# sara-nl/2D-VQ-AE-2

Hardware: AMD Instinct MI355X
Metric: patches/sec (VQAE.forward: encoder -> VQ -> decoder) (higher is better)
Workload: dtype f32; 1 GPU; BASELINE configs[1] (cfg B): batch 256/GPU of 256x256x3 fp32 -> 32x32 codes, K=256, D=128, full forward; global_batch=256, parallelism=patch-sharded x1

## Files before the change

### 2d-vq-ae-2_amd/csrc/conv_wino.hip

```cpp
#include "kernels.h"
#include "mfma.h"

namespace {

using namespace vqae;

struct WinoK {
    const float* __restrict__ t1;
    const float* __restrict__ U;
    const float* __restrict__ w3;
    const float* __restrict__ w1n;
    float* xio;
    float* y2;
    int H, Wimg, M;
    float act_a, act_b, t_scale, t_b4, n_b1a, n_b1b, n_b2a, n_b2b;
};

constexpr int BPF = 6;

template <int C> struct WinoCfg {
    static constexpr int W = C >= 128 ? 32 : (C == 64 ? 64 : 128);
    static constexpr int NT = C == 256 ? 512 : 256;
    static constexpr int NW = NT / 64;
    static constexpr int PX = 4 * W;
    static constexpr int TILES = PX / 4;
    static constexpr int TC = W / 2;
    static constexpr int NS = C / 32;
    static constexpr int KS = C / 8;
    static constexpr int C4 = C / 4;
    static constexpr int RP = NT / C4;
    static constexpr int LDT = C + 4;
    static constexpr int NI = C >= 64 ? 2 : 1;
    static constexpr int WN = C / (32 * NI);
    static constexpr int MI = PX / ((NW / WN) * 32);
    static constexpr int LDS_BYTES = PX * LDT * 4;
    static constexpr int PREF = C <= 64 ? 1 : 0;
};

template <int C, int TAIL, int DT, bool WIDE>
__global__ __launch_bounds__((WinoCfg<C>::NT), 2)
void wino_trunk_kernel(const WinoK p) {
    using K = WinoCfg<C>;
    auto rnd = [](float v) -> float {
        if (DT == VQAE_DT_BF16) return (float)(__bf16)v;
        if (DT == VQAE_DT_F16) return (float)(_Float16)v;
        return v;
    };
    auto rnd4 = [&](f32x4 v) -> f32x4 {
        if (DT != VQAE_DT_F32) {
#pragma unroll
            for (int e = 0; e < 4; ++e) v[e] = rnd(v[e]);
        }
        return v;
    };
    constexpr int W = K::W, PX = K::PX, TC = K::TC, NS = K::NS, KS = K::KS, C4 = K::C4, RP = K::RP, LDT = K::LDT, WN = K::WN;
    constexpr int MI = K::MI, NI = K::NI;
    constexpr bool PREF = K::PREF && !WIDE;
// ... 57 lines not shown
        for (int s_c = 0; s_c < 2; ++s_c)
#pragma unroll
            for (int j = 0; j < 4; ++j)
                v[2 * s_r + s_c][j] = xi == 1 ? la[s_c][j] + lb[s_c][j] : la[s_c][j] - lb[s_c][j];
    };
    tr_load(0, 0);
    tr_combine(0, 0);
    tr_load(0, 1);
    tr_combine(0, 1);

    const int wm = wave / WN, wn = wave % WN;
    const int64_t pix0 = ((int64_t)img * p.H + row0) * Wimg + col0 + tj0;
    float* xr[4];
    f32x4 res[16];
    f32x4 bt[2][4][NI];
    auto tail_prefetch = [&](const float* __restrict__ wsrc) {
        const float* b0 = wsrc + (wn * NI) * (KS * 256) + 4 * lane;
#pragma unroll
        for (int u = 0; u < 4; ++u)
#pragma unroll
            for (int ni = 0; ni < NI; ++ni) bt[0][u][ni] = *reinterpret_cast<const f32x4*>(b0 + ni * (KS * 256) + 256 * u);
    };

    f32x16 y00, y01, y10, y11;
#pragma unroll
    for (int r = 0; r < 16; ++r) { y00[r] = 0.f; y01[r] = 0.f; y10[r] = 0.f; y11[r] = 0.f; }
#pragma unroll
    for (int xi = 0; xi < 4; ++xi) {
        __builtin_amdgcn_sched_barrier(0);
        if (xi > 0) __syncthreads();
#pragma unroll
        for (int it = 0; it < 4; ++it) {
            const int tile = (it >> 1) * TC + tj0 + RP * (it & 1);
            float* dst = lds + tile * LDT + 4 * cg;
            *reinterpret_cast<f32x4*>(dst + 0 * K::TILES * LDT) = v[it][0] - v[it][2];
            *reinterpret_cast<f32x4*>(dst + 1 * K::TILES * LDT) = v[it][1] + v[it][2];
            *reinterpret_cast<f32x4*>(dst + 2 * K::TILES * LDT) = v[it][2] - v[it][1];
            *reinterpret_cast<f32x4*>(dst + 3 * K::TILES * LDT) = v[it][1] - v[it][3];
        }

        const float* const ux = ub + (int64_t)(4 * xi) * (C * C);
#define WB(s) (((s) / KS) * (C * C) + 256 * ((s) % KS))
        f32x4 bq[BPF];
#pragma unroll
        for (int s = 0; s < BPF; ++s)
            bq[s] = *reinterpret_cast<const f32x4*>(ux + WB(s));
        __syncthreads();
        if (PREF && xi < 3) tr_load(xi + 1, 0);
        f32x4 aq[2];
        aq[0] = *reinterpret_cast<const f32x4*>(af);
#pragma unroll
        for (int nu = 0; nu < 4; ++nu) {
            f32x16 acc;
#pragma unroll
            for (int r = 0; r < 16; ++r) acc[r] = 0.f;
#pragma unroll
            for (int u = 0; u < KS; ++u) {
                const int s = KS * nu + u;
                if (s + 1 < STEPS)
                    aq[(s + 1) & 1] = *reinterpret_cast<const f32x4*>(af + ((s + 1) / KS) * K::TILES * LDT + 8 * ((s + 1) % KS));
                const f32x4 b = bq[s % BPF];
                if (s + BPF < STEPS)
                    bq[s % BPF] = *reinterpret_cast<const f32x4*>(ux + WB(s + BPF));
                if (xi == 3 && s == STEPS - BPF) {
                    tail_prefetch(p.w3);
#pragma unroll
                    for (int r = 0; r < 4; ++r) xr[r] = p.xio + (pix0 + (int64_t)r * Wimg) * C + 4 * cg;
#pragma unroll
                    for (int i = 0; i < 16; ++i) res[i] = __builtin_nontemporal_load(reinterpret_cast<const f32x4*>(xr[(RP * i) / W] + ((RP * i) % W) * C));
                }
#pragma unroll
                for (int r = 0; r < 4; ++r)
                    acc = __builtin_amdgcn_mfma_f32_32x32x2f32(b[r], aq[s & 1][r], acc, 0, 0, 0);
                __builtin_amdgcn_sched_barrier(0);
            }
            const int ca0 = xi <= 2 ? 1 : 0, ca1 = xi == 0 ? 0 : (xi == 1 ? 1 : -1);
            const int cb0 = nu <= 2 ? 1 : 0, cb1 = nu == 0 ? 0 : (nu == 1 ? 1 : -1);
            if (ca0 * cb0 != 0) y00 = y00 + acc;
            if (ca0 * cb1 == 1) y01 = y01 + acc; else if (ca0 * cb1 == -1) y01 = y01 - acc;
            if (ca1 * cb0 == 1) y10 = y10 + acc; else if (ca1 * cb0 == -1) y10 = y10 - acc;
            if (ca1 * cb1 == 1) y11 = y11 + acc; else if (ca1 * cb1 == -1) y11 = y11 - acc;
            asm volatile("" : "+v"(y00), "+v"(y01), "+v"(y10), "+v"(y11));
        }
#undef WB
        if (xi < 3) {
            if (!PREF) tr_load(xi + 1, 0);
            tr_combine(xi + 1, 0); tr_load(xi + 1, 1); tr_combine(xi + 1, 1);
        }
    }

    __syncthreads();
    float* const T = lds;
    {
        const int tile = mt * 32 + li;
        const int px = (2 * (tile / TC)) * W + 2 * (tile % TC);
        float* const d = T + px * LDT + 32 * ns + 4 * hh;
#pragma unroll
        for (int g = 0; g < 4; ++g) {
            f32x4 o00, o01, o10, o11;
#pragma unroll
            for (int e = 0; e < 4; ++e) {
                o00[e] = rnd(elu_act(rnd(y00[4 * g + e]) + p.act_a) + p.act_b);
                o01[e] = rnd(elu_act(rnd(y01[4 * g + e]) + p.act_a) + p.act_b);
                o10[e] = rnd(elu_act(rnd(y10[4 * g + e]) + p.act_a) + p.act_b);
// ... 4 lines not shown
            *reinterpret_cast<f32x4*>(d + 8 * g + W * LDT) = o10;
            *reinterpret_cast<f32x4*>(d + 8 * g + (W + 1) * LDT) = o11;
        }
    }
    __syncthreads();

    f32x16 acc[MI][NI];
    auto gemm_tail = [&](const float* __restrict__ wsrc) {
#pragma unroll
        for (int mi = 0; mi < MI; ++mi)
#pragma unroll
            for (int ni = 0; ni < NI; ++ni)
#pragma unroll
                for (int r = 0; r < 16; ++r) acc[mi][ni][r] = 0.f;
        const float* a0 = T + (wm * MI * 32 + li) * LDT + 4 * hh;
        const float* b0 = wsrc + (wn * NI) * (KS * 256) + 4 * lane;
        f32x4 a[2][MI];
#pragma unroll
        for (int mi = 0; mi < MI; ++mi) a[0][mi] = *reinterpret_cast<const f32x4*>(a0 + mi * 32 * LDT);
#pragma unroll
        for (int ug = 0; ug < KS / 4; ++ug) {
            if (ug + 1 < KS / 4) {
#pragma unroll
                for (int u = 0; u < 4; ++u)
#pragma unroll
                    for (int ni = 0; ni < NI; ++ni)
                        bt[(ug + 1) & 1][u][ni] = *reinterpret_cast<const f32x4*>(b0 + ni * (KS * 256) + 256 * (4 * (ug + 1) + u));
            }
#pragma unroll
            for (int u = 0; u < 4; ++u) {
// ... 256 lines not shown
#pragma unroll
    for (int a = 0; a < 4; ++a) {
        U[(a * 4 + 0) * cc + fo] = t[a][0];
        U[(a * 4 + 1) * cc + fo] = 0.5f * (t[a][0] + t[a][1] + t[a][2]);
        U[(a * 4 + 2) * cc + fo] = 0.5f * (t[a][0] - t[a][1] + t[a][2]);
        U[(a * 4 + 3) * cc + fo] = t[a][2];
    }
}

__global__ void frag_weight_kernel(const float* __restrict__ w, int n_rows, int K, int sk, float* __restrict__ out) {
    const int i = blockIdx.x * blockDim.x + threadIdx.x;
    if (i >= n_rows * K) return;
    out[frag_offset(i / K, i % K, K, sk)] = w[i];
}

template <int C, int DT, bool WIDE>
int launch_wino_w(const WinoK& k, bool chain, hipStream_t stream) {
    using K = WinoCfg<C>;
    if (int rc = vqae::set_max_dynamic_lds((const void*)wino_trunk_kernel<C, 1, DT, WIDE>, K::LDS_BYTES)) return rc;
    if (int rc = vqae::set_max_dynamic_lds((const void*)wino_trunk_kernel<C, 2, DT, WIDE>, K::LDS_BYTES)) return rc;
    const unsigned grid = (unsigned)(k.M / K::PX);
    const double flops = 2.0 * (double)k.M * C * (4.0 * C + C + (chain ? C : 0));
    vqae::ProfScope prof(C >= 128 ? vqae::PROF_CONV3X3_TRUNK : vqae::PROF_NONE, stream, flops);
    if (chain) wino_trunk_kernel<C, 2, DT, WIDE><<<grid, K::NT, K::LDS_BYTES, stream>>>(k);
    else wino_trunk_kernel<C, 1, DT, WIDE><<<grid, K::NT, K::LDS_BYTES, stream>>>(k);
    prof.done();
    VQAE_LAUNCH_CHECK();
    return VQAE_OK;
}

template <int C, int DT = VQAE_DT_F32>
int launch_wino(const WinoK& k, bool chain, hipStream_t stream) {
    return k.Wimg == WinoCfg<C>::W ? launch_wino_w<C, DT, false>(k, chain, stream) : launch_wino_w<C, DT, true>(k, chain, stream);
}

}

namespace vqae {

bool wino_trunk_channels(int c, int dtype) { return dtype == VQAE_DT_F32 ? (c == 256 || c == 128 || c == 64 || c == 32) : c == 32; }

bool wino_trunk_supported(int c, int h, int w, int dtype) {
    if (!wino_trunk_channels(c, dtype)) return false;
    const int span = c >= 128 ? 32 : (c == 64 ? WinoCfg<64>::W : WinoCfg<32>::W);
    return w >= span && w % span == 0 && h >= 4 && h % 4 == 0;
}

size_t wino_weight_floats(int c) { return (size_t)16 * c * c; }

int wino_transform_weight(const float* w_oihw_dev, int c, int dtype, float* U_dev, hipStream_t stream) {
    wino_weight_kernel<<<(unsigned)ceil_div(c * c, 256), 256, 0, stream>>>(w_oihw_dev, c, dtype, U_dev);
    VQAE_LAUNCH_CHECK();
    return VQAE_OK;
}

bool fixup_conv1_supported(int c, int64_t m) {
    if (c != 256 && c != 128 && c != 64 && c != 32) return false;
    const int px = c >= 128 ? 128 : (c == 64 ? WinoCfg<64>::PX : WinoCfg<32>::PX);
    return m > 0 && m % px == 0;
}

template <int C>
static int launch_conv1(const float* x, const float* w1f, float pa, float pb, float aa, float ab, float* y, int64_t m,
// ... 23 lines not shown
    VQAE_REQUIRE(m / 128 < (1ll << 31), VQAE_ERR_UNSUPPORTED, "fixup_conv1: too many pixels");
    if (c == 256) return launch_conv1<256>(x, w1f, pa, pb, aa, ab, y, m, stream);
    if (c == 128) return launch_conv1<128>(x, w1f, pa, pb, aa, ab, y, m, stream);
    if (c == 64) return launch_conv1<64>(x, w1f, pa, pb, aa, ab, y, m, stream);
    return launch_conv1<32>(x, w1f, pa, pb, aa, ab, y, m, stream);
}

int frag_weight(const float* w_packed_dev, int n_rows, int K, int sk, float* out_dev, hipStream_t stream) {
    VQAE_REQUIRE(n_rows % 32 == 0 && (sk == 8 || sk == 16) && K % sk == 0, VQAE_ERR_INVALID, "frag_weight: %d x %d, k-slice %d", n_rows, K, sk);
    frag_weight_kernel<<<(unsigned)ceil_div((int64_t)n_rows * K, 256), 256, 0, stream>>>(w_packed_dev, n_rows, K, sk, out_dev);
    VQAE_LAUNCH_CHECK();
    return VQAE_OK;
}

int wino_trunk_tail(const float* t1, const float* U, const float* w3, float act_a, float act_b, float t_scale, float t_b4,
                    float* xio, const NextConv1& next, int batch, int h, int w, int c, int dtype, hipStream_t stream) {
    if (batch == 0) return VQAE_OK;
    const float* w1n = (const float*)next.w1;
    float* t1_next = (float*)next.t1_next;
    VQAE_REQUIRE(t1 && U && w3 && xio && (!w1n || t1_next), VQAE_ERR_INVALID, "wino_trunk_tail: null pointer");
    VQAE_REQUIRE(wino_trunk_supported(c, h, w, dtype), VQAE_ERR_UNSUPPORTED, "wino_trunk_tail: C = %d, H = %d, W = %d, dtype %d", c, h, w, dtype);
    const int64_t M = (int64_t)batch * h * w;
    VQAE_REQUIRE(M < (1ll << 31) - 256, VQAE_ERR_UNSUPPORTED, "wino_trunk_tail: too many pixels");
    WinoK k;
    memset(&k, 0, sizeof(k));
    k.t1 = t1; k.U = U; k.w3 = w3; k.w1n = w1n; k.xio = xio; k.y2 = t1_next;
    k.H = h; k.Wimg = w; k.M = (int)M;
    k.act_a = act_a; k.act_b = act_b; k.t_scale = t_scale; k.t_b4 = t_b4;
    k.n_b1a = next.b1a; k.n_b1b = next.b1b; k.n_b2a = next.b2a; k.n_b2b = next.b2b;
    return dtype == VQAE_DT_BF16 ? launch_wino<32, VQAE_DT_BF16>(k, w1n != nullptr, stream)
         : dtype == VQAE_DT_F16 ? launch_wino<32, VQAE_DT_F16>(k, w1n != nullptr, stream)
         : c == 256 ? launch_wino<256>(k, w1n != nullptr, stream)
         : c == 128 ? launch_wino<128>(k, w1n != nullptr, stream)
         : (c == 64 ? launch_wino<64>(k, w1n != nullptr, stream) : launch_wino<32>(k, w1n != nullptr, stream));
}

}
```

### 2d-vq-ae-2_amd/csrc/handle.hip

```cpp
#include "kernels.h"

#include <algorithm>
#include <cmath>
#include <cstdlib>
#include <map>
#include <mutex>
#include <set>
#include <string>
#include <unordered_map>
#include <utility>
#include <vector>

namespace vqae {
char* last_error_buf() {
    static thread_local char buf[512] = {0};
    return buf;
}

ProfState& prof_state() {
    static ProfState p;
    return p;
}

int set_max_dynamic_lds(const void* kernel, int bytes) {
// ... 60 lines not shown
}

extern "C" const char* vqae_last_error(void) { return vqae::last_error_buf(); }
extern "C" const char* vqae_build_info(void) { return "gfx950;fp32-mfma;" __DATE__; }

namespace {

enum { MODE_SAME = 0, MODE_DOWN = 1, MODE_UP = 2 };

struct Block : vqae::FixupScalars {
    int mode, cin, cout, br;
    float *w1, *w2, *w3, *wskip;
    float* wU43 = nullptr;
    void *wU43s = nullptr, *w1s = nullptr, *w3s = nullptr;
    float* wU = nullptr;
    float *w1f = nullptr, *w3f = nullptr;
    float *w2f = nullptr, *wskf = nullptr;
    void *w1h = nullptr, *w2h = nullptr, *w3h = nullptr, *wskh = nullptr;
    int kind = VQAE_BLOCK_FIXUP, hidden = 0;
    float *bv1 = nullptr, *bv2 = nullptr, *bv3 = nullptr;
    float *fc0w = nullptr, *fc0b = nullptr, *fc2w = nullptr, *fc2b = nullptr;
};

const float kMean255[3] = {0.7279f * 255.0f, 0.5955f * 255.0f, 0.7762f * 255.0f};
const float kInv255[3] = {1.0f / (0.2419f * 255.0f), 1.0f / (0.3083f * 255.0f), 1.0f / (0.1741f * 255.0f)};
const float kStd255[3] = {0.2419f * 255.0f, 0.3083f * 255.0f, 0.1741f * 255.0f};

}

struct vqae_handle {
// ... 12 lines not shown
    size_t buf_floats = 0;
    void* vq_ws = nullptr;
    size_t vq_ws_bytes = 0;
    float* loss_scratch = nullptr;
    int device = 0;
    bool has_encoder = false, has_decoder = false;
    bool fuse_trunk = true;
    bool t1_ready = false;
    bool up_conv_first = true;
    bool fuse_down = true;
    bool fuse_down16 = true;
    bool fuse_up16 = true;
    bool fuse_up_tail = true;
    bool use_wino = true;
    bool w43_split = true;
    void* idx_scratch = nullptr;
    size_t idx_scratch_bytes = 0;
    float* se_ws = nullptr;
    size_t se_ws_bytes = 0;
    size_t se_gate_off = 0;
};

namespace {

using TensorMap = std::unordered_map<std::string, const vqae_tensor*>;

int find(const TensorMap& tm, const std::string& name, int64_t numel, const float** out) {
    auto it = tm.find(name);
    if (it == tm.end()) return vqae::fail(VQAE_ERR_NOT_FOUND, "missing tensor '%s'", name.c_str());
    if (it->second->numel != numel)
// ... 65 lines not shown
    return VQAE_OK;
}

int load_block(vqae_handle* h, const TensorMap& tm, const std::string& pre, int mode, int cin, int cout, Block* b) {
    *b = Block();
    b->mode = mode; b->cin = cin; b->cout = cout; b->br = cin > cout ? cin : cout;
    const int dt = h->cfg.compute_dtype;
    const bool f32 = dt == VQAE_DT_F32, same = mode == MODE_SAME && cout == cin;
    int rc;
#define S_(field, nm) if ((rc = scalar(tm, pre + "." nm, &b->field))) return rc;
    S_(b1a, "bias1a") S_(b1b, "bias1b") S_(b2a, "bias2a") S_(b2b, "bias2b") S_(b3a, "bias3a") S_(b3b, "bias3b")
    S_(b4, "bias4") S_(scale, "scale")
    const bool wino = same && h->use_wino && vqae::wino_trunk_channels(cin, dt);
    const bool wino43 = wino && f32 && vqae::wino43_enabled() && vqae::wino43_channels(cin);
    const bool split = wino43 && h->w43_split && vqae::wino43_split_supported(cin);
    const bool tail = wino || (same && vqae::conv_trunk_tail_channels(cin));
    const bool trunk16 = same && !f32 && vqae::trunk16_channels(cin);
    const bool same8 = same && !f32 && vqae::same8_16_channels(cin);
    const bool down = mode == MODE_DOWN && cout == 2 * cin && h->fuse_down && vqae::down_block_channels(cin);
    const bool down16 = mode == MODE_DOWN && cout == 2 * cin && !f32 && h->fuse_down16 && vqae::down16_channels(cin);
    const bool up16 = mode == MODE_UP && cin == 2 * cout && !f32 && h->fuse_up16 && vqae::up16_channels(cin);

    const int k2 = mode == MODE_SAME ? 3 : (mode == MODE_DOWN ? 2 : 1);
    const float* p;
    if ((rc = find(tm, pre + ".branch_conv1.weight", (int64_t)b->br * cin, &p))) return rc;
    if ((rc = upload_packed(h, p, b->br, cin, 1, &b->w1))) return rc;
    if ((rc = find(tm, pre + ".branch_conv2.weight", (int64_t)b->br * b->br * k2 * k2, &p))) return rc;
    if ((rc = upload_packed(h, p, b->br, b->br, k2, &b->w2))) return rc;
    if (wino && (rc = upload_wino(h, p, cin, &b->wU))) return rc;
    if (wino43 && (rc = upload_wino43(h, p, cin, false, (void**)&b->wU43))) return rc;
    if (split && (rc = upload_wino43(h, p, cin, true, &b->wU43s))) return rc;
    if ((rc = find(tm, pre + ".branch_conv3.weight", (int64_t)cout * b->br, &p))) return rc;
    if ((rc = upload_packed(h, p, cout, b->br, 1, &b->w3))) return rc;
    if (mode != MODE_SAME) {
        S_(b1c, "bias1c") S_(b1d, "bias1d")
        const int ks = mode == MODE_DOWN ? 2 : 1;
        if ((rc = find(tm, pre + ".skip_conv.weight", (int64_t)cout * cin * ks * ks, &p))) return rc;
        if ((rc = upload_packed(h, p, cout, cin, ks, &b->wskip))) return rc;
    }
#undef S_
    auto frag = [&](const float* src, int rows, int K, int sk, float** dst) {
        if (int r = dev_alloc(h, (size_t)rows * K * 4, (void**)dst)) return r;
        return vqae::frag_weight(src, rows, K, sk, *dst, nullptr);
    };
    auto frag_tail = [&](const float* src, float** dst) {
        return frag(src, cin, cin, wino ? 8 : vqae::conv_tail_kslice(dt, cin), dst);
    };
    auto frag_rect = [&](const float* src, int K, float** dst) { return frag(src, cout, K, 8, dst); };
    auto split3 = [&](const float* src, void** dst) {
        if (int r = dev_alloc(h, vqae::split_1x1_bytes(cin), dst)) return r;
        return vqae::split_1x1_weight(src, cin, *dst, nullptr);
    };
    auto pack_t16 = [&](const float* src, int taps, void** dst) {
        if (int r = dev_alloc(h, vqae::trunk16_weight_bytes(cin, taps), dst)) return r;
        return vqae::pack16_weight(src, cin, taps * cin, dt, *dst, nullptr);
    };
    auto pack_r16 = [&](const float* src, int rows, int K, void** dst) {
        if (int r = dev_alloc(h, vqae::down16_weight_bytes(rows, K), dst)) return r;
        return vqae::pack16_weight(src, rows, K, dt, *dst, nullptr);
    };
    if (tail && ((rc = frag_tail(b->w1, &b->w1f)) || (rc = frag_tail(b->w3, &b->w3f)))) return rc;
    if (split && ((rc = split3(b->w1, &b->w1s)) || (rc = split3(b->w3, &b->w3s)))) return rc;
    if (trunk16 && ((rc = pack_t16(b->w1, 1, &b->w1h)) || (rc = pack_t16(b->w2, 9, &b->w2h)) || (rc = pack_t16(b->w3, 1, &b->w3h)))) return rc;
    if (same8 && ((rc = pack_r16(b->w2, 8, 72, &b->w2h)) || (rc = pack_r16(b->w3, 8, 8, &b->w3h)))) return rc;
    if (down && ((rc = frag_rect(b->w1, cin, &b->w1f)) || (rc = frag_rect(b->w2, 4 * cout, &b->w2f)) ||
                 (rc = frag_rect(b->w3, cout, &b->w3f)) || (rc = frag_rect(b->wskip, 4 * cin, &b->wskf)))) return rc;
    if (down16 && ((rc = pack_r16(b->w1, cout, cin, &b->w1h)) || (rc = pack_r16(b->w2, cout, 4 * cout, &b->w2h)) ||
                   (rc = pack_r16(b->w3, cout, cout, &b->w3h)) || (rc = pack_r16(b->wskip, cout, 4 * cin, &b->wskh)))) return rc;
    if (up16 && ((rc = pack_t16(b->w1, 1, &b->w1h)) || (rc = pack_r16(b->w2, cin, cin, &b->w2h)) ||
                 (rc = pack_r16(b->w3, cout, cin, &b->w3h)) || (rc = pack_r16(b->wskip, cout, cin, &b->wskh)))) return rc;
    VQAE_HIP_CHECK(hipDeviceSynchronize());
    return VQAE_OK;
}

int bn_fold(const TensorMap& tm, const std::string& pre, int c, float eps, std::vector<float>* g, std::vector<float>* shift) {
    const float *gamma, *beta, *mean, *var;
    int rc;
// ... 127 lines not shown
    if ((rc = vqae_dwconv_f32(P, b.w2, b.bv2, B, H, W, E, dwm, 1, Q, partial, st))) return rc;
    if ((rc = vqae_se_gate_f32(partial, B, Ho, Wo, E, b.fc0w, b.fc0b, b.hidden, b.fc2w, b.fc2b, gate, st))) return rc;
    ConvCall c3(h, B, Ho, Wo, E, b.cout, 1, 1, 0, VQAE_PAD_NONE);
    c3.a.pre_mode = VQAE_PRE_CHANNEL_GATE;
    float* out = skip == X ? X : R;
    if ((rc = vqae_conv2d_gated_f32(&c3.a, Q, gate, b.w3, b.bv3, skip, out, st))) return rc;
    if (out == R) std::swap(h->buf[0], h->buf[3]);
    H = Ho; W = Wo;
    return VQAE_OK;
}

enum Route {
    R_SAME16_16,
    R_TRUNK16,
    R_WINO43_SPLIT, R_WINO43,
    R_WINO,
    R_TAIL,
    R_SAME8_16,
    R_FIXUP_FUSED,
    R_SAME,
    R_DOWN16, R_DOWN_FUSED, R_DOWN,
    R_UP_CONV_FIRST_TAIL,
    R_UP_CONV_FIRST,
    R_UP16,
    R_UP
};

bool same_width_next(const Block& b, const Block* next) {
    return next && next->mode == MODE_SAME && next->cin == b.cin && next->cout == b.cin;
}

Route select_route(const vqae_handle* h, const Block& b, const Block* next, int B, int H, int W) {
    const int dt = h->cfg.compute_dtype;
    const bool f32 = dt == VQAE_DT_F32;
    if (b.mode == MODE_SAME) {
        if (b.w2h && h->fuse_trunk && vqae::same16_16_supported(b.cin, H, W, dt)) return R_SAME16_16;
        if (b.w2h && h->fuse_trunk && vqae::trunk16_supported(b.cin, H, W, dt)) return R_TRUNK16;
        if (b.wU && h->fuse_trunk && vqae::wino_trunk_supported(b.cin, H, W, dt)) {
            if (!(b.wU43 && vqae::wino43_supported(b.cin, H, W, dt))) return R_WINO;
            const bool chain = same_width_next(b, next) && next->w1f;
            return b.wU43s && (!chain || next->w1s) ? R_WINO43_SPLIT : R_WINO43;
        }
        if (vqae::conv_trunk_tail_channels(b.cin) && b.cout == b.cin && h->fuse_trunk) return R_TAIL;
        if (b.w2h && !f32 && vqae::same8_16_supported(b.cin, H, W, dt)) return R_SAME8_16;
        if (b.cin == b.cout && vqae_fixup_same_supported(b.cin, H, W)) return R_FIXUP_FUSED;
        return R_SAME;
    }
    if (b.mode == MODE_DOWN) {
        if (b.w2h && !f32 && vqae::down16_supported(b.cin, H, W)) return R_DOWN16;
        if (b.w2f && vqae::down_block_supported(b.cin, H, W)) return R_DOWN_FUSED;
        return R_DOWN;
    }
    if (f32 && h->up_conv_first) return h->fuse_up_tail && vqae::up_tail_supported(b.br, b.cout) ? R_UP_CONV_FIRST_TAIL : R_UP_CONV_FIRST;
    if (b.w2h && vqae::up16_supported(b.cin, H, W, dt) && vqae::trunk16_head_supported(b.cin, (int64_t)B * H * W, dt)) return R_UP16;
    return R_UP;
}

int run_conv1(const vqae_handle* h, const Block& b, int B, int H, int W, const float* x, float* y, hipStream_t st) {
    return conv(ConvCall(h, B, H, W, b.cin, b.br, 1, 1, 0, VQAE_PAD_NONE).pre(VQAE_PRE_BIAS_ELU_BIAS, b.b1a, b.b1b).act(b.b2a, b.b2b), x, b.w1, nullptr, y, st);
}

int run_trunk(vqae_handle* h, Route r, const Block& b, const Block* next, int B, int H, int W, hipStream_t st) {
    float *X = h->buf[0], *P = h->buf[1], *Q = h->buf[2];
    const int dt = h->cfg.compute_dtype;
    const int64_t M = (int64_t)B * H * W;
    const bool t16 = r == R_TRUNK16, wino = r == R_WINO43_SPLIT || r == R_WINO43 || r == R_WINO;
    int rc;
    if (!h->t1_ready) {
        if (t16 && vqae::trunk16_head_supported(b.cin, M, dt)) {
            rc = vqae::trunk16_head(X, b.w1h, b.b1a, b.b1b, b.b2a, b.b2b, P, M, b.cin, dt, false, st);
        } else if (t16) {
            if ((rc = run_conv1(h, b, B, H, W, X, Q, st))) return rc;
            rc = vqae::trunk16_round_pack(Q, P, M * b.cin, dt, st);
        } else if (wino && dt == VQAE_DT_F32 && vqae::fixup_conv1_supported(b.cin, M)) {
            rc = vqae::fixup_conv1(X, b.w1f, b.b1a, b.b1b, b.b2a, b.b2b, P, M, b.cin, st);
        } else {
            rc = run_conv1(h, b, B, H, W, X, P, st);
        }
        if (rc) return rc;
    }
    vqae::NextConv1 nx;
    const void* next_w1 = !same_width_next(b, next) ? nullptr : (t16 ? next->w1h : (const void*)next->w1f);
    if (next_w1) nx = {next_w1, next->w1s, next->b1a, next->b1b, next->b2a, next->b2b, Q};
    if (t16) {
        rc = vqae::trunk16_block(P, b.w2h, b.w3h, b.b3a, b.b3b, b.scale, b.b4, X, nx, B, H, W, b.cin, dt, st);
    } else if (r == R_WINO43_SPLIT || r == R_WINO43) {
        rc = vqae::wino43_trunk_tail(P, b.wU43, b.w3f, b.b3a, b.b3b, b.scale, b.b4, X, nx, B, H, W, b.cin, st,
                                     r == R_WINO43_SPLIT ? b.wU43s : nullptr, b.w3s);
    } else if (r == R_WINO) {
        rc = vqae::wino_trunk_tail(P, b.wU, b.w3f, b.b3a, b.b3b, b.scale, b.b4, X, nx, B, H, W, b.cin, dt, st);
    } else {
        const ConvCall c2 = ConvCall(h, B, H, W, b.br, b.br, 3, 1, 1, VQAE_PAD_CIRCULAR).act(b.b3a, b.b3b);
        rc = vqae::conv_trunk_tail(&c2.a, P, b.w2, b.w3f, b.scale, b.b4, X, nx, st);
    }
    if (rc) return rc;
    if (nx.w1) std::swap(h->buf[1], h->buf[2]);
    h->t1_ready = nx.w1 != nullptr;
    return VQAE_OK;
}

int run_block(vqae_handle* h, const Block& b, const Block* next, int B, int& H, int& W, hipStream_t st) {
    if (b.kind == VQAE_BLOCK_MBCONV) return run_mbconv(h, b, B, H, W, st);
    float *X = h->buf[0], *P = h->buf[1], *Q = h->buf[2], *R = h->buf[3];
    const int dt = h->cfg.compute_dtype;
    const Route r = select_route(h, b, next, B, H, W);
// ... 228 lines not shown
    if (cfg->block_kind == VQAE_BLOCK_MBCONV) {
        VQAE_REQUIRE(cfg->compute_dtype == VQAE_DT_F32, VQAE_ERR_UNSUPPORTED, "MBConv blocks run in fp32 only");
        VQAE_REQUIRE(cfg->expand_ratio >= 1 && cfg->se_divisor >= 1 && cfg->bn_eps > 0.f, VQAE_ERR_INVALID,
                     "MBConv: expand_ratio %d, se_divisor %d, bn_eps %g", cfg->expand_ratio, cfg->se_divisor, (double)cfg->bn_eps);
    }
    TensorMap tm;
    for (int i = 0; i < n_tensors; ++i) tm[tensors[i].name] = &tensors[i];

    vqae_handle* h = new vqae_handle();
    h->cfg = *cfg;
    if (hipGetDevice(&h->device) != hipSuccess) { delete h; return vqae::fail(VQAE_ERR_HIP, "hipGetDevice failed"); }
    h->fuse_trunk = vqae::env_int("VQAE_NO_TRUNK_FUSION", 0) == 0;
    h->up_conv_first = vqae::env_int("VQAE_NO_UP_REORDER", 0) == 0;
    h->use_wino = vqae::env_int("VQAE_NO_WINOGRAD", 0) == 0;
    h->w43_split = vqae::env_int("VQAE_W43_SPLIT", 1) != 0;
    h->fuse_up_tail = vqae::env_int("VQAE_NO_UP_TAIL_FUSION", 0) == 0;
    h->fuse_down = vqae::env_int("VQAE_NO_DOWN_FUSION", 0) == 0;
    h->fuse_down16 = vqae::env_int("VQAE_NO_DOWN16", 0) == 0;
    h->fuse_up16 = vqae::env_int("VQAE_NO_UP16", 0) == 0;
    h->fuse_stem16 = vqae::env_int("VQAE_NO_STEM16", 0) == 0;
    h->fuse_vq = vqae::env_int("VQAE_NO_VQ_FUSION", 0) == 0;
    h->C = cfg->stem << cfg->n_down;
    h->D = cfg->projection_dim > 0 ? cfg->projection_dim : h->C;
    h->K = cfg->num_embeddings;
    int rc = VQAE_OK;
    const float* p;
    auto bail = [&](int code) { vqae_destroy(h); return code; };

    const bool has_enc = tm.count("encoder.in_stem.weight") > 0;
    const bool has_dec = tm.count("decoder.out_stem.weight") > 0;
// ... 318 lines not shown
```

### 2d-vq-ae-2_amd/csrc/kernels.h

```cpp
#pragma once
#include "common.h"

namespace vqae {

struct FixupScalars {
    float b1a, b1b, b2a, b2b, b3a, b3b, b4, scale, b1c, b1d;
};
static_assert(sizeof(FixupScalars) == 10 * sizeof(float), "FixupScalars is read as float[8] / float[10]");

struct NextConv1 {
    const void* w1 = nullptr;
    const void* w1s = nullptr;
    float b1a = 0.f, b1b = 0.f, b2a = 0.f, b2b = 0.f;
    void* t1_next = nullptr;
};

bool conv_trunk_tail_channels(int c);
int conv_tail_kslice(int dtype, int cin);
int conv_trunk_tail(const vqae_conv_args* a, const float* t1, const float* w2, const float* w3, float t_scale, float t_b4,
                    float* xio, const NextConv1& next, hipStream_t stream);

bool wino_trunk_channels(int c, int dtype);
bool wino_trunk_supported(int c, int h, int w, int dtype);
size_t wino_weight_floats(int c);
int wino_transform_weight(const float* w_oihw_dev, int c, int dtype, float* U_dev, hipStream_t stream);
int frag_weight(const float* w_packed_dev, int n_rows, int K, int sk, float* out_dev, hipStream_t stream);
int wino_trunk_tail(const float* t1, const float* U, const float* w3, float act_a, float act_b, float t_scale, float t_b4,
                    float* xio, const NextConv1& next, int batch, int h, int w, int c, int dtype, hipStream_t stream);
bool fixup_conv1_supported(int c, int64_t m);
int fixup_conv1(const float* x, const float* w1f, float pa, float pb, float aa, float ab, float* y, int64_t m, int c,
                hipStream_t stream);

bool wino43_channels(int c);
bool wino43_supported(int c, int h, int w, int dtype);
bool wino43_enabled();
size_t wino43_weight_floats(int c);
int wino43_transform_weight(const float* w_oihw_dev, int c, float* U_dev, hipStream_t stream);
bool wino43_split_supported(int c);
size_t wino43_split_weight_bytes(int c);
size_t split_1x1_bytes(int c);
int wino43_split_weight(const float* w_oihw_dev, int c, void* U_dev, hipStream_t stream);
int split_1x1_weight(const float* w_packed_dev, int c, void* out_dev, hipStream_t stream);
int wino43_trunk_tail(const float* t1, const float* U, const float* w3, float act_a, float act_b, float t_scale, float t_b4,
// ... 76 lines not shown
```

Before: 4247 patches/s.

## Emulate fp32 Winograd trunk GEMMs for C=32 with three-way bf16 split MFMAs

Adds a split-precision path for the C=32 Winograd residual trunk kernel. Weights are pre-split on device into three bf16 planes, activations are split on the fly, and each fp32 32x32x2 MFMA chain is replaced by six 32x32x16 bf16 MFMAs that drop the low-order cross terms. The 1x1 tail and next-conv weights are split the same way. The aim is to use the much higher bf16 matrix throughput while keeping near-fp32 accuracy. The cost is extra VALU work for splitting activations and slightly different rounding. The path is on by default, with an environment variable to disable it.

```diff
diff --git a/2d-vq-ae-2_amd/csrc/conv_wino.hip b/2d-vq-ae-2_amd/csrc/conv_wino.hip
--- a/2d-vq-ae-2_amd/csrc/conv_wino.hip
+++ b/2d-vq-ae-2_amd/csrc/conv_wino.hip
@@ -15,6 +15,27 @@
     int H, Wimg, M;
     float act_a, act_b, t_scale, t_b4, n_b1a, n_b1b, n_b2a, n_b2b;
 };
+
+__device__ __forceinline__ f32x4 widen(const bf16x4& b) {
+    const u32x2 u = __builtin_bit_cast(u32x2, b);
+    const u32x4 w = {u[0] << 16, u[0] & 0xffff0000u, u[1] << 16, u[1] & 0xffff0000u};
+    return __builtin_bit_cast(f32x4, w);
+}
+__device__ __forceinline__ void split3(const f32x4& v, bf16x4 (&h)[3]) {
+    h[0] = __builtin_convertvector(v, bf16x4);
+    const f32x4 r1 = v - widen(h[0]);
+    h[1] = __builtin_convertvector(r1, bf16x4);
+    const f32x4 r2 = r1 - widen(h[1]);
+    h[2] = __builtin_convertvector(r2, bf16x4);
+}
+__device__ __forceinline__ void split3x8(const f32x4& v0, const f32x4& v1, bf16x8 (&x)[3]) {
+    bf16x4 lo[3], hi[3];
+    split3(v0, lo);
+    split3(v1, hi);
+#pragma unroll
+    for (int pl = 0; pl < 3; ++pl) x[pl] = __builtin_shufflevector(lo[pl], hi[pl], 0, 1, 2, 3, 4, 5, 6, 7);
+}
+__device__ __forceinline__ bf16x8 as_bf8(const f32x4& v) { return __builtin_bit_cast(bf16x8, v); }
 
 constexpr int BPF = 6;
 
@@ -37,10 +58,11 @@
     static constexpr int PREF = C <= 64 ? 1 : 0;
 };
 
-template <int C, int TAIL, int DT, bool WIDE>
+template <int C, int TAIL, int DT, bool WIDE, bool SPLIT = false>
 __global__ __launch_bounds__((WinoCfg<C>::NT), 2)
 void wino_trunk_kernel(const WinoK p) {
     using K = WinoCfg<C>;
+    static_assert(!SPLIT || (C == 32 && DT == VQAE_DT_F32 && !WIDE), "split form: C = 32, fp32, exact-width grid");
     auto rnd = [](float v) -> float {
         if (DT == VQAE_DT_BF16) return (float)(__bf16)v;
         if (DT == VQAE_DT_F16) return (float)(_Float16)v;
@@ -128,7 +150,13 @@
     float* xr[4];
     f32x4 res[16];
     f32x4 bt[2][4][NI];
+    f32x4 bts[3 * KS / 2];
     auto tail_prefetch = [&](const float* __restrict__ wsrc) {
+        if constexpr (SPLIT) {
+#pragma unroll
+            for (int f = 0; f < 3 * KS / 2; ++f) bts[f] = *reinterpret_cast<const f32x4*>(wsrc + 256 * f + 4 * lane);
+            return;
+        }
         const float* b0 = wsrc + (wn * NI) * (KS * 256) + 4 * lane;
 #pragma unroll
         for (int u = 0; u < 4; ++u)
@@ -139,6 +167,15 @@
     f32x16 y00, y01, y10, y11;
 #pragma unroll
     for (int r = 0; r < 16; ++r) { y00[r] = 0.f; y01[r] = 0.f; y10[r] = 0.f; y11[r] = 0.f; }
+#define FOLD(xi, nu, acc) { \
+        const int ca0 = xi <= 2 ? 1 : 0, ca1 = xi == 0 ? 0 : (xi == 1 ? 1 : -1); \
+        const int cb0 = nu <= 2 ? 1 : 0, cb1 = nu == 0 ? 0 : (nu == 1 ? 1 : -1); \
+        if (ca0 * cb0 != 0) y00 = y00 + acc; \
+        if (ca0 * cb1 == 1) y01 = y01 + acc; else if (ca0 * cb1 == -1) y01 = y01 - acc; \
+        if (ca1 * cb0 == 1) y10 = y10 + acc; else if (ca1 * cb0 == -1) y10 = y10 - acc; \
+        if (ca1 * cb1 == 1) y11 = y11 + acc; else if (ca1 * cb1 == -1) y11 = y11 - acc; \
+        asm volatile("" : "+v"(y00), "+v"(y01), "+v"(y10), "+v"(y11)); \
+    }
 #pragma unroll
     for (int xi = 0; xi < 4; ++xi) {
         __builtin_amdgcn_sched_barrier(0);
@@ -153,55 +190,102 @@
             *reinterpret_cast<f32x4*>(dst + 3 * K::TILES * LDT) = v[it][1] - v[it][3];
         }
 
-        const float* const ux = ub + (int64_t)(4 * xi) * (C * C);
+        if constexpr (SPLIT) {
+            const float* const ux = p.U + (4 * xi) * (3 * C * C / 2) + 4 * lane;
+#define WB(f) (((f) / 6) * (3 * C * C / 2) + 256 * ((f) % 6))
+            f32x4 bq[6];
+#pragma unroll
+            for (int f = 0; f < 6; ++f) bq[f] = *reinterpret_cast<const f32x4*>(ux + WB(f));
+            __syncthreads();
+            if (PREF && xi < 3) tr_load(xi + 1, 0);
+            f32x4 aq[2][2];
+            aq[0][0] = *reinterpret_cast<const f32x4*>(af);
+            aq[0][1] = *reinterpret_cast<const f32x4*>(af + 8);
+#pragma unroll
+            for (int nu = 0; nu < 4; ++nu) {
+                f32x16 acc;
+#pragma unroll
+                for (int r = 0; r < 16; ++r) acc[r] = 0.f;
+#pragma unroll
+                for (int t = 0; t < 2; ++t) {
+                    const int s = 2 * nu + t;
+                    if (s + 1 < 8) {
+                        aq[(s + 1) & 1][0] = *reinterpret_cast<const f32x4*>(af + ((s + 1) / 2) * K::TILES * LDT + 16 * ((s + 1) % 2));
+                        aq[(s + 1) & 1][1] = *reinterpret_cast<const f32x4*>(af + ((s + 1) / 2) * K::TILES * LDT + 16 * ((s + 1) % 2) + 8);
+                    }
+                    if (xi == 3 && s == 6) {
+                        tail_prefetch(p.w3);
+#pragma unroll
+                        for (int r = 0; r < 4; ++r) xr[r] = p.xio + (pix0 + (int64_t)r * Wimg) * C + 4 * cg;
+#pragma unroll
+                        for (int i = 0; i < 16; ++i) res[i] = __builtin_nontemporal_load(reinterpret_cast<const f32x4*>(xr[(RP * i) / W] + ((RP * i) % W) * C));
+                    }
+                    bf16x8 x[3];
+                    split3x8(aq[s & 1][0], aq[s & 1][1], x);
+#define MM(f, pb) acc = __builtin_amdgcn_mfma_f32_32x32x16_bf16(as_bf8(bq[3 * t + (f)]), x[pb], acc, 0, 0, 0)
+#define RELOAD(f) if (nu < 3) bq[3 * t + (f)] = *reinterpret_cast<const f32x4*>(ux + WB(6 * (nu + 1) + 3 * t + (f)))
+                    MM(1, 1);
+                    MM(1, 0);
+                    RELOAD(1);
+                    MM(2, 0);
+                    RELOAD(2);
+                    MM(0, 2);
+                    MM(0, 1);
+                    MM(0, 0);
+                    RELOAD(0);
+#undef MM
+#undef RELOAD
+                    __builtin_amdgcn_sched_barrier(0);
+                }
+                FOLD(xi, nu, acc)
+            }
+#undef WB
+        } else {
+            const float* const ux = ub + (int64_t)(4 * xi) * (C * C);
 #define WB(s) (((s) / KS) * (C * C) + 256 * ((s) % KS))
-        f32x4 bq[BPF];
-#pragma unroll
-        for (int s = 0; s < BPF; ++s)
-            bq[s] = *reinterpret_cast<const f32x4*>(ux + WB(s));
-        __syncthreads();
-        if (PREF && xi < 3) tr_load(xi + 1, 0);
-        f32x4 aq[2];
-        aq[0] = *reinterpret_cast<const f32x4*>(af);
-#pragma unroll
-        for (int nu = 0; nu < 4; ++nu) {
-            f32x16 acc;
-#pragma unroll
-            for (int r = 0; r < 16; ++r) acc[r] = 0.f;
-#pragma unroll
-            for (int u = 0; u < KS; ++u) {
-                const int s = KS * nu + u;
-                if (s + 1 < STEPS)
-                    aq[(s + 1) & 1] = *reinterpret_cast<const f32x4*>(af + ((s + 1) / KS) * K::TILES * LDT + 8 * ((s + 1) % KS));
-                const f32x4 b = bq[s % BPF];
-                if (s + BPF < STEPS)
-                    bq[s % BPF] = *reinterpret_cast<const f32x4*>(ux + WB(s + BPF));
-                if (xi == 3 && s == STEPS - BPF) {
-                    tail_prefetch(p.w3);
-#pragma unroll
-                    for (int r = 0; r < 4; ++r) xr[r] = p.xio + (pix0 + (int64_t)r * Wimg) * C + 4 * cg;
-#pragma unroll
-                    for (int i = 0; i < 16; ++i) res[i] = __builtin_nontemporal_load(reinterpret_cast<const f32x4*>(xr[(RP * i) / W] + ((RP * i) % W) * C));
+            f32x4 bq[BPF];
+#pragma unroll
+            for (int s = 0; s < BPF; ++s)
+                bq[s] = *reinterpret_cast<const f32x4*>(ux + WB(s));
+            __syncthreads();
+            if (PREF && xi < 3) tr_load(xi + 1, 0);
+            f32x4 aq[2];
+            aq[0] = *reinterpret_cast<const f32x4*>(af);
+#pragma unroll
+            for (int nu = 0; nu < 4; ++nu) {
+                f32x16 acc;
+#pragma unroll
+                for (int r = 0; r < 16; ++r) acc[r] = 0.f;
+#pragma unroll
+                for (int u = 0; u < KS; ++u) {
+                    const int s = KS * nu + u;
+                    if (s + 1 < STEPS)
+                        aq[(s + 1) & 1] = *reinterpret_cast<const f32x4*>(af + ((s + 1) / KS) * K::TILES * LDT + 8 * ((s + 1) % KS));
+                    const f32x4 b = bq[s % BPF];
+                    if (s + BPF < STEPS)
+                        bq[s % BPF] = *reinterpret_cast<const f32x4*>(ux + WB(s + BPF));
+                    if (xi == 3 && s == STEPS - BPF) {
+                        tail_prefetch(p.w3);
+#pragma unroll
+                        for (int r = 0; r < 4; ++r) xr[r] = p.xio + (pix0 + (int64_t)r * Wimg) * C + 4 * cg;
+#pragma unroll
+                        for (int i = 0; i < 16; ++i) res[i] = __builtin_nontemporal_load(reinterpret_cast<const f32x4*>(xr[(RP * i) / W] + ((RP * i) % W) * C));
+                    }
+#pragma unroll
+                    for (int r = 0; r < 4; ++r)
+                        acc = __builtin_amdgcn_mfma_f32_32x32x2f32(b[r], aq[s & 1][r], acc, 0, 0, 0);
+                    __builtin_amdgcn_sched_barrier(0);
                 }
-#pragma unroll
-                for (int r = 0; r < 4; ++r)
-                    acc = __builtin_amdgcn_mfma_f32_32x32x2f32(b[r], aq[s & 1][r], acc, 0, 0, 0);
-                __builtin_amdgcn_sched_barrier(0);
-            }
-            const int ca0 = xi <= 2 ? 1 : 0, ca1 = xi == 0 ? 0 : (xi == 1 ? 1 : -1);
-            const int cb0 = nu <= 2 ? 1 : 0, cb1 = nu == 0 ? 0 : (nu == 1 ? 1 : -1);
-            if (ca0 * cb0 != 0) y00 = y00 + acc;
-            if (ca0 * cb1 == 1) y01 = y01 + acc; else if (ca0 * cb1 == -1) y01 = y01 - acc;
-            if (ca1 * cb0 == 1) y10 = y10 + acc; else if (ca1 * cb0 == -1) y10 = y10 - acc;
-            if (ca1 * cb1 == 1) y11 = y11 + acc; else if (ca1 * cb1 == -1) y11 = y11 - acc;
-            asm volatile("" : "+v"(y00), "+v"(y01), "+v"(y10), "+v"(y11));
-        }
+                FOLD(xi, nu, acc)
+            }
 #undef WB
+        }
         if (xi < 3) {
             if (!PREF) tr_load(xi + 1, 0);
             tr_combine(xi + 1, 0); tr_load(xi + 1, 1); tr_combine(xi + 1, 1);
         }
     }
+#undef FOLD
 
     __syncthreads();
     float* const T = lds;
@@ -236,6 +320,26 @@
 #pragma unroll
                 for (int r = 0; r < 16; ++r) acc[mi][ni][r] = 0.f;
         const float* a0 = T + (wm * MI * 32 + li) * LDT + 4 * hh;
+        if constexpr (SPLIT) {
+#pragma unroll
+            for (int t = 0; t < KS / 2; ++t) {
+                bf16x8 x[MI][3];
+#pragma unroll
+                for (int mi = 0; mi < MI; ++mi)
+                    split3x8(*reinterpret_cast<const f32x4*>(a0 + mi * 32 * LDT + 16 * t),
+                             *reinterpret_cast<const f32x4*>(a0 + mi * 32 * LDT + 16 * t + 8), x[mi]);
+#define MM(f, pb) for (int mi = 0; mi < MI; ++mi) \
+                    acc[mi][0] = __builtin_amdgcn_mfma_f32_32x32x16_bf16(as_bf8(bts[3 * t + (f)]), x[mi][pb], acc[mi][0], 0, 0, 0)
+                MM(1, 1);
+                MM(1, 0);
+                MM(2, 0);
+                MM(0, 2);
+                MM(0, 1);
+                MM(0, 0);
+#undef MM
+            }
+            return;
+        }
         const float* b0 = wsrc + (wn * NI) * (KS * 256) + 4 * lane;
         f32x4 a[2][MI];
 #pragma unroll
@@ -522,16 +626,63 @@
     out[frag_offset(i / K, i % K, K, sk)] = w[i];
 }
 
-template <int C, int DT, bool WIDE>
+__device__ void split3_f64(double v, __bf16 (&h)[3]) {
+    for (int pl = 0; pl < 3; ++pl) {
+        h[pl] = (__bf16)(float)v;
+        v -= (double)(float)h[pl];
+    }
+}
+
+__device__ __forceinline__ int split_offset(int n, int k, int K) {
+    return ((n >> 5) * (K / 16) + (k >> 4)) * 1536 + (((k >> 2) & 1) * 32 + (n & 31)) * 8 + ((k >> 3) & 1) * 4 + (k & 3);
+}
+
+__global__ void wino_split_weight_kernel(const float* __restrict__ w, int c, __bf16* __restrict__ U) {
+    const int i = blockIdx.x * blockDim.x + threadIdx.x;
+    if (i >= c * c) return;
+    double g[3][3], t[4][3], u[16];
+    for (int a = 0; a < 3; ++a)
+        for (int b = 0; b < 3; ++b) g[a][b] = (double)w[(int64_t)i * 9 + a * 3 + b];
+    for (int b = 0; b < 3; ++b) {
+        t[0][b] = g[0][b];
+        t[1][b] = 0.5 * (g[0][b] + g[1][b] + g[2][b]);
+        t[2][b] = 0.5 * (g[0][b] - g[1][b] + g[2][b]);
+        t[3][b] = g[2][b];
+    }
+    for (int a = 0; a < 4; ++a) {
+        u[a * 4 + 0] = t[a][0];
+        u[a * 4 + 1] = 0.5 * (t[a][0] + t[a][1] + t[a][2]);
+        u[a * 4 + 2] = 0.5 * (t[a][0] - t[a][1] + t[a][2]);
+        u[a * 4 + 3] = t[a][2];
+    }
+    const int fo = split_offset(i / c, i % c, c);
+    const int64_t cc3 = (int64_t)3 * c * c;
+    for (int x = 0; x < 16; ++x) {
+        __bf16 h[3];
+        split3_f64(u[x], h);
+        for (int pl = 0; pl < 3; ++pl) U[x * cc3 + fo + pl * 512] = h[pl];
+    }
+}
+
+__global__ void wino_split_1x1_kernel(const float* __restrict__ w, int c, __bf16* __restrict__ out) {
+    const int i = blockIdx.x * blockDim.x + threadIdx.x;
+    if (i >= c * c) return;
+    __bf16 h[3];
+    split3_f64((double)w[i], h);
+    const int fo = split_offset(i / c, i % c, c);
+    for (int pl = 0; pl < 3; ++pl) out[fo + pl * 512] = h[pl];
+}
+
+template <int C, int DT, bool WIDE, bool SPLIT = false>
 int launch_wino_w(const WinoK& k, bool chain, hipStream_t stream) {
     using K = WinoCfg<C>;
-    if (int rc = vqae::set_max_dynamic_lds((const void*)wino_trunk_kernel<C, 1, DT, WIDE>, K::LDS_BYTES)) return rc;
-    if (int rc = vqae::set_max_dynamic_lds((const void*)wino_trunk_kernel<C, 2, DT, WIDE>, K::LDS_BYTES)) return rc;
+    if (int rc = vqae::set_max_dynamic_lds((const void*)wino_trunk_kernel<C, 1, DT, WIDE, SPLIT>, K::LDS_BYTES)) return rc;
+    if (int rc = vqae::set_max_dynamic_lds((const void*)wino_trunk_kernel<C, 2, DT, WIDE, SPLIT>, K::LDS_BYTES)) return rc;
     const unsigned grid = (unsigned)(k.M / K::PX);
     const double flops = 2.0 * (double)k.M * C * (4.0 * C + C + (chain ? C : 0));
     vqae::ProfScope prof(C >= 128 ? vqae::PROF_CONV3X3_TRUNK : vqae::PROF_NONE, stream, flops);
-    if (chain) wino_trunk_kernel<C, 2, DT, WIDE><<<grid, K::NT, K::LDS_BYTES, stream>>>(k);
-    else wino_trunk_kernel<C, 1, DT, WIDE><<<grid, K::NT, K::LDS_BYTES, stream>>>(k);
+    if (chain) wino_trunk_kernel<C, 2, DT, WIDE, SPLIT><<<grid, K::NT, K::LDS_BYTES, stream>>>(k);
+    else wino_trunk_kernel<C, 1, DT, WIDE, SPLIT><<<grid, K::NT, K::LDS_BYTES, stream>>>(k);
     prof.done();
     VQAE_LAUNCH_CHECK();
     return VQAE_OK;
@@ -555,6 +706,27 @@
 }
 
 size_t wino_weight_floats(int c) { return (size_t)16 * c * c; }
+
+bool wino_split_channels(int c) { return c == 32; }
+bool wino_split_supported(int c, int h, int w, int dtype) {
+    return dtype == VQAE_DT_F32 && wino_split_channels(c) && w == WinoCfg<32>::W && wino_trunk_supported(c, h, w, dtype);
+}
+size_t wino_split_weight_bytes(int c) { return (size_t)16 * c * c * 3 * 2; }
+size_t wino_split_1x1_bytes(int c) { return (size_t)c * c * 3 * 2; }
+
+int wino_split_weight(const float* w_oihw_dev, int c, void* Us_dev, hipStream_t stream) {
+    VQAE_REQUIRE(wino_split_channels(c), VQAE_ERR_UNSUPPORTED, "wino_split_weight: C = %d", c);
+    wino_split_weight_kernel<<<(unsigned)ceil_div(c * c, 256), 256, 0, stream>>>(w_oihw_dev, c, (__bf16*)Us_dev);
+    VQAE_LAUNCH_CHECK();
+    return VQAE_OK;
+}
+
+int wino_split_1x1_weight(const float* w_packed_dev, int c, void* out_dev, hipStream_t stream) {
+    VQAE_REQUIRE(wino_split_channels(c), VQAE_ERR_UNSUPPORTED, "wino_split_1x1_weight: C = %d", c);
+    wino_split_1x1_kernel<<<(unsigned)ceil_div(c * c, 256), 256, 0, stream>>>(w_packed_dev, c, (__bf16*)out_dev);
+    VQAE_LAUNCH_CHECK();
+    return VQAE_OK;
+}
 
 int wino_transform_weight(const float* w_oihw_dev, int c, int dtype, float* U_dev, hipStream_t stream) {
     wino_weight_kernel<<<(unsigned)ceil_div(c * c, 256), 256, 0, stream>>>(w_oihw_dev, c, dtype, U_dev);
@@ -608,7 +780,8 @@
 }
 
 int wino_trunk_tail(const float* t1, const float* U, const float* w3, float act_a, float act_b, float t_scale, float t_b4,
-                    float* xio, const NextConv1& next, int batch, int h, int w, int c, int dtype, hipStream_t stream) {
+                    float* xio, const NextConv1& next, int batch, int h, int w, int c, int dtype, hipStream_t stream,
+                    const void* Us, const void* w3s) {
     if (batch == 0) return VQAE_OK;
     const float* w1n = (const float*)next.w1;
     float* t1_next = (float*)next.t1_next;
@@ -622,6 +795,12 @@
     k.H = h; k.Wimg = w; k.M = (int)M;
     k.act_a = act_a; k.act_b = act_b; k.t_scale = t_scale; k.t_b4 = t_b4;
     k.n_b1a = next.b1a; k.n_b1b = next.b1b; k.n_b2a = next.b2a; k.n_b2b = next.b2b;
+    if (Us) {
+        VQAE_REQUIRE(wino_split_supported(c, h, w, dtype) && w3s && (!w1n || next.w1s), VQAE_ERR_INVALID,
+                     "wino_trunk_tail: the split form needs C = 32 on the 128-wide fp32 grid and its three weights");
+        k.U = (const float*)Us; k.w3 = (const float*)w3s; k.w1n = (const float*)next.w1s;
+        return launch_wino_w<32, VQAE_DT_F32, false, true>(k, w1n != nullptr, stream);
+    }
     return dtype == VQAE_DT_BF16 ? launch_wino<32, VQAE_DT_BF16>(k, w1n != nullptr, stream)
          : dtype == VQAE_DT_F16 ? launch_wino<32, VQAE_DT_F16>(k, w1n != nullptr, stream)
          : c == 256 ? launch_wino<256>(k, w1n != nullptr, stream)
diff --git a/2d-vq-ae-2_amd/csrc/handle.hip b/2d-vq-ae-2_amd/csrc/handle.hip
--- a/2d-vq-ae-2_amd/csrc/handle.hip
+++ b/2d-vq-ae-2_amd/csrc/handle.hip
@@ -98,6 +98,7 @@
     float* wU43 = nullptr;
     void *wU43s = nullptr, *w1s = nullptr, *w3s = nullptr;
     float* wU = nullptr;
+    void* wUs = nullptr;
     float *w1f = nullptr, *w3f = nullptr;
     float *w2f = nullptr, *wskf = nullptr;
     void *w1h = nullptr, *w2h = nullptr, *w3h = nullptr, *wskh = nullptr;
@@ -140,6 +141,7 @@
     bool fuse_up_tail = true;
     bool use_wino = true;
     bool w43_split = true;
+    bool w32_split = true;
     void* idx_scratch = nullptr;
     size_t idx_scratch_bytes = 0;
     float* se_ws = nullptr;
@@ -235,6 +237,7 @@
     const bool wino = same && h->use_wino && vqae::wino_trunk_channels(cin, dt);
     const bool wino43 = wino && f32 && vqae::wino43_enabled() && vqae::wino43_channels(cin);
     const bool split = wino43 && h->w43_split && vqae::wino43_split_supported(cin);
+    const bool split32 = wino && f32 && h->w32_split && vqae::wino_split_channels(cin);
     const bool tail = wino || (same && vqae::conv_trunk_tail_channels(cin));
     const bool trunk16 = same && !f32 && vqae::trunk16_channels(cin);
     const bool same8 = same && !f32 && vqae::same8_16_channels(cin);
@@ -249,6 +252,8 @@
     if ((rc = find(tm, pre + ".branch_conv2.weight", (int64_t)b->br * b->br * k2 * k2, &p))) return rc;
     if ((rc = upload_packed(h, p, b->br, b->br, k2, &b->w2))) return rc;
     if (wino && (rc = upload_wino(h, p, cin, &b->wU))) return rc;
+    if (split32 && (rc = upload_via(h, p, (size_t)cin * cin * 9 * 4, vqae::wino_split_weight_bytes(cin), "winograd weight transform",
+                                    [=](const float* raw, void* U) { return vqae::wino_split_weight(raw, cin, U, nullptr); }, &b->wUs))) return rc;
     if (wino43 && (rc = upload_wino43(h, p, cin, false, (void**)&b->wU43))) return rc;
     if (split && (rc = upload_wino43(h, p, cin, true, &b->wU43s))) return rc;
     if ((rc = find(tm, pre + ".branch_conv3.weight", (int64_t)cout * b->br, &p))) return rc;
@@ -272,6 +277,10 @@
         if (int r = dev_alloc(h, vqae::split_1x1_bytes(cin), dst)) return r;
         return vqae::split_1x1_weight(src, cin, *dst, nullptr);
     };
+    auto split3_32 = [&](const float* src, void** dst) {
+        if (int r = dev_alloc(h, vqae::wino_split_1x1_bytes(cin), dst)) return r;
+        return vqae::wino_split_1x1_weight(src, cin, *dst, nullptr);
+    };
     auto pack_t16 = [&](const float* src, int taps, void** dst) {
         if (int r = dev_alloc(h, vqae::trunk16_weight_bytes(cin, taps), dst)) return r;
         return vqae::pack16_weight(src, cin, taps * cin, dt, *dst, nullptr);
@@ -282,6 +291,7 @@
     };
     if (tail && ((rc = frag_tail(b->w1, &b->w1f)) || (rc = frag_tail(b->w3, &b->w3f)))) return rc;
     if (split && ((rc = split3(b->w1, &b->w1s)) || (rc = split3(b->w3, &b->w3s)))) return rc;
+    if (split32 && ((rc = split3_32(b->w1, &b->w1s)) || (rc = split3_32(b->w3, &b->w3s)))) return rc;
     if (trunk16 && ((rc = pack_t16(b->w1, 1, &b->w1h)) || (rc = pack_t16(b->w2, 9, &b->w2h)) || (rc = pack_t16(b->w3, 1, &b->w3h)))) return rc;
     if (same8 && ((rc = pack_r16(b->w2, 8, 72, &b->w2h)) || (rc = pack_r16(b->w3, 8, 8, &b->w3h)))) return rc;
     if (down && ((rc = frag_rect(b->w1, cin, &b->w1f)) || (rc = frag_rect(b->w2, 4 * cout, &b->w2f)) ||
@@ -439,7 +449,7 @@
     R_SAME16_16,
     R_TRUNK16,
     R_WINO43_SPLIT, R_WINO43,
-    R_WINO,
+    R_WINO_SPLIT, R_WINO,
     R_TAIL,
     R_SAME8_16,
     R_FIXUP_FUSED,
@@ -462,8 +472,9 @@
         if (b.w2h && h->fuse_trunk && vqae::same16_16_supported(b.cin, H, W, dt)) return R_SAME16_16;
         if (b.w2h && h->fuse_trunk && vqae::trunk16_supported(b.cin, H, W, dt)) return R_TRUNK16;
         if (b.wU && h->fuse_trunk && vqae::wino_trunk_supported(b.cin, H, W, dt)) {
-            if (!(b.wU43 && vqae::wino43_supported(b.cin, H, W, dt))) return R_WINO;
             const bool chain = same_width_next(b, next) && next->w1f;
+            if (!(b.wU43 && vqae::wino43_supported(b.cin, H, W, dt)))
+                return b.wUs && b.w3s && (!chain || next->w1s) && vqae::wino_split_supported(b.cin, H, W, dt) ? R_WINO_SPLIT : R_WINO;
             return b.wU43s && (!chain || next->w1s) ? R_WINO43_SPLIT : R_WINO43;
         }
         if (vqae::conv_trunk_tail_channels(b.cin) && b.cout == b.cin && h->fuse_trunk) return R_TAIL;
@@ -489,7 +500,7 @@
     float *X = h->buf[0], *P = h->buf[1], *Q = h->buf[2];
     const int dt = h->cfg.compute_dtype;
     const int64_t M = (int64_t)B * H * W;
-    const bool t16 = r == R_TRUNK16, wino = r == R_WINO43_SPLIT || r == R_WINO43 || r == R_WINO;
+    const bool t16 = r == R_TRUNK16, wino = r == R_WINO43_SPLIT || r == R_WINO43 || r == R_WINO_SPLIT || r == R_WINO;
     int rc;
     if (!h->t1_ready) {
         if (t16 && vqae::trunk16_head_supported(b.cin, M, dt)) {
@@ -512,8 +523,9 @@
     } else if (r == R_WINO43_SPLIT || r == R_WINO43) {
         rc = vqae::wino43_trunk_tail(P, b.wU43, b.w3f, b.b3a, b.b3b, b.scale, b.b4, X, nx, B, H, W, b.cin, st,
                                      r == R_WINO43_SPLIT ? b.wU43s : nullptr, b.w3s);
-    } else if (r == R_WINO) {
-        rc = vqae::wino_trunk_tail(P, b.wU, b.w3f, b.b3a, b.b3b, b.scale, b.b4, X, nx, B, H, W, b.cin, dt, st);
+    } else if (r == R_WINO_SPLIT || r == R_WINO) {
+        rc = vqae::wino_trunk_tail(P, b.wU, b.w3f, b.b3a, b.b3b, b.scale, b.b4, X, nx, B, H, W, b.cin, dt, st,
+                                   r == R_WINO_SPLIT ? b.wUs : nullptr, b.w3s);
     } else {
         const ConvCall c2 = ConvCall(h, B, H, W, b.br, b.br, 3, 1, 1, VQAE_PAD_CIRCULAR).act(b.b3a, b.b3b);
         rc = vqae::conv_trunk_tail(&c2.a, P, b.w2, b.w3f, b.scale, b.b4, X, nx, st);
@@ -772,6 +784,7 @@
     h->up_conv_first = vqae::env_int("VQAE_NO_UP_REORDER", 0) == 0;
     h->use_wino = vqae::env_int("VQAE_NO_WINOGRAD", 0) == 0;
     h->w43_split = vqae::env_int("VQAE_W43_SPLIT", 1) != 0;
+    h->w32_split = vqae::env_int("VQAE_W32_SPLIT", 1) != 0;
     h->fuse_up_tail = vqae::env_int("VQAE_NO_UP_TAIL_FUSION", 0) == 0;
     h->fuse_down = vqae::env_int("VQAE_NO_DOWN_FUSION", 0) == 0;
     h->fuse_down16 = vqae::env_int("VQAE_NO_DOWN16", 0) == 0;
diff --git a/2d-vq-ae-2_amd/csrc/kernels.h b/2d-vq-ae-2_amd/csrc/kernels.h
--- a/2d-vq-ae-2_amd/csrc/kernels.h
+++ b/2d-vq-ae-2_amd/csrc/kernels.h
@@ -26,7 +26,14 @@
 int wino_transform_weight(const float* w_oihw_dev, int c, int dtype, float* U_dev, hipStream_t stream);
 int frag_weight(const float* w_packed_dev, int n_rows, int K, int sk, float* out_dev, hipStream_t stream);
 int wino_trunk_tail(const float* t1, const float* U, const float* w3, float act_a, float act_b, float t_scale, float t_b4,
-                    float* xio, const NextConv1& next, int batch, int h, int w, int c, int dtype, hipStream_t stream);
+                    float* xio, const NextConv1& next, int batch, int h, int w, int c, int dtype, hipStream_t stream,
+                    const void* Us = nullptr, const void* w3s = nullptr);
+bool wino_split_channels(int c);
+bool wino_split_supported(int c, int h, int w, int dtype);
+size_t wino_split_weight_bytes(int c);
+size_t wino_split_1x1_bytes(int c);
+int wino_split_weight(const float* w_oihw_dev, int c, void* Us_dev, hipStream_t stream);
+int wino_split_1x1_weight(const float* w_packed_dev, int c, void* out_dev, hipStream_t stream);
 bool fixup_conv1_supported(int c, int64_t m);
 int fixup_conv1(const float* x, const float* w1f, float pa, float pb, float aa, float ab, float* y, int64_t m, int c,
                 hipStream_t stream);
```

New measurement: 4277 patches/s, median of 6. No clear change (+0.7%).
